# toonsegers/verifiable_mpc

Hardware: AMD Instinct MI355X
Metric: Ed25519 MSM scalar-mults/sec (higher is better)
Workload: dtype u32 (255-bit modular integers as 10 limbs of 25.5 bits, 32x32->64 multiply-adds)

## Files before the change

verifiable_mpc_amd/csrc/api.hip:

```cpp
#include <stdlib.h>

#include "common.h"


thread_local char vmpc_err_buf[512] = {0};

__attribute__((constructor)) static void vmpc_hw_queues_default() { setenv("GPU_MAX_HW_QUEUES", "16", 0); }

int vmpc_fr_check_dev(vmpc_ctx *ctx, const void *v, size_t n);

extern "C" const char *vmpc_last_error(void) { return vmpc_err_buf; }

const char *vmpc_getenv_experimental(const char *name) {
    const char *on = getenv("VMPC_EXPERIMENTAL");
    return (on && atoi(on) != 0) ? getenv(name) : nullptr;
}

extern "C" int vmpc_backend_info(char *buf, size_t buflen) {
    int n = 0;
    hipError_t e = hipGetDeviceCount(&n);
    if (e != hipSuccess || n <= 0) {
        if (buf && buflen) snprintf(buf, buflen, "no HIP device (%s)", hipGetErrorString(e));
        return VMPC_E_NODEV;
    }
// ... 16 lines not shown
        snprintf(vmpc_err_buf, sizeof vmpc_err_buf, "no HIP device visible");
        return VMPC_E_NODEV;
    }
    if (device < 0 || device >= n) return VMPC_E_INVAL;
    VMPC_HIP_CHECK(hipSetDevice(device));
    vmpc_ctx *c = new vmpc_ctx();
    c->device = device;
    hipDeviceProp_t p;
    if (hipGetDeviceProperties(&p, device) == hipSuccess) {
        c->cu_count = p.multiProcessorCount;
        c->lds_optin = p.sharedMemPerBlockOptin ? p.sharedMemPerBlockOptin : p.sharedMemPerBlock;
    }
    hipError_t e = hipStreamCreateWithFlags(&c->stream, hipStreamNonBlocking);
    if (e != hipSuccess) {
        delete c;
        snprintf(vmpc_err_buf, sizeof vmpc_err_buf, "hipStreamCreate: %s", hipGetErrorString(e));
        return VMPC_E_HIP;
    }
    c->own_stream = true;
    e = hipMalloc((void **)&c->d_status, (VMPC_ST_WORDS + 16) * sizeof(uint32_t));
    if (e == hipSuccess) e = hipMemset(c->d_status, 0, (VMPC_ST_WORDS + 16) * sizeof(uint32_t));
    if (e != hipSuccess) {
        VMPC_IGNORE(hipStreamDestroy(c->stream));
        delete c;
        snprintf(vmpc_err_buf, sizeof vmpc_err_buf, "hipMalloc(status): %s", hipGetErrorString(e));
        return VMPC_E_HIP;
    }
    const char *w = getenv("VMPC_MSM_WINDOW");
    if (w) c->window_override = atoi(w);
    const char *fj = getenv("VMPC_FOLD_JUMP_DIGITS");
    if (fj && atoi(fj) == 4) c->fold_jump_digit_bits = 4;
    const char *sp = getenv("VMPC_SHORT_PATH");
    if (sp) c->short_path = atoi(sp) != 0;
    const char *bb = vmpc_getenv_experimental("VMPC_BUCKET_BLOCK");
    if (bb && atoi(bb) == 1024) c->bucket_block = 1024;
    const char *bw = vmpc_getenv_experimental("VMPC_BUCKET_WGS_PER_CU");
    if (bw && atoi(bw) >= 0) c->bucket_wgs_per_cu = atoi(bw);
    const char *sf = vmpc_getenv_experimental("VMPC_SORT_FINE_BITS");
    if (sf && atoi(sf) >= 0) c->sort_fine_bits = atoi(sf);
    const char *rc = vmpc_getenv_experimental("VMPC_REDUCE_MAX_CHUNKS");
    if (rc && atoi(rc) >= 256 && atoi(rc) <= 32768) c->reduce_max_chunks = atoi(rc);
    const char *ro = vmpc_getenv_experimental("VMPC_REDUCE_CHUNKS");
    if (ro && atoi(ro) >= 64 && atoi(ro) <= 32768 && (atoi(ro) & (atoi(ro) - 1)) == 0) c->reduce_chunks_override = atoi(ro);
    const char *rt = vmpc_getenv_experimental("VMPC_REDUCE_TREE");
    if (rt) c->reduce_tree = atoi(rt) != 0;
    const char *ss = vmpc_getenv_experimental("VMPC_SEG_SHIFT_MIN");
    if (ss && atoi(ss) <= 0 && atoi(ss) >= -5) c->seg_shift_min = atoi(ss);
    *out = c;
    return VMPC_OK;
}

extern "C" int vmpc_ctx_destroy(vmpc_ctx *ctx) {
    if (!ctx) return VMPC_E_INVAL;
    if (ctx->p4_pool_busy) {
        snprintf(vmpc_err_buf, sizeof vmpc_err_buf, "vmpc_ctx_destroy: a vmpc_p4 of this context is still alive");
        return VMPC_E_INVAL;
    }
    VMPC_IGNORE(hipSetDevice(ctx->device));
    VMPC_IGNORE(hipStreamSynchronize(ctx->stream));
    for (auto &s : ctx->stages)
        for (auto &pr : s.pending) {
            VMPC_IGNORE(hipEventDestroy(pr.first));
            VMPC_IGNORE(hipEventDestroy(pr.second));
        }
    for (auto e : ctx->event_pool) VMPC_IGNORE(hipEventDestroy(e));
    if (ctx->xevent) VMPC_IGNORE(hipEventDestroy(ctx->xevent));
    if (ctx->ev_sorted) VMPC_IGNORE(hipEventDestroy(ctx->ev_sorted));
    if (ctx->ev_bucketed) VMPC_IGNORE(hipEventDestroy(ctx->ev_bucketed));
// ... 431 lines not shown
```

verifiable_mpc_amd/csrc/bn256_impl.h:

```cpp
#pragma once
#include "common.h"
#include "msm_sort.h"
#include "sw256.h"
#include "bn256_curve.h"

#define BN_B2A_CANON                                                                           \
    { 0xdb6c6949u, 0x7774124bu, 0x96e598bbu, 0x5a0cdfc5u, 0x111033b1u, 0x90e7f281u, 0x1aa5abfbu,  \
      0x64984e1fu }
#define BN_B2B_CANON                                                                           \
    { 0xd6340f0au, 0x35a2de0au, 0x83455ef6u, 0x316f8daeu, 0x7026e2d0u, 0x5dd7fe12u, 0xbaa9f3ffu,  \
      0x0e5ee696u }
static const msm_modulus BN_ORDER = {{0x57ac7261u, 0x1a2ef45bu, 0xf82b3924u, 0x2e8d8e12u, 0x6184dc21u,
                                      0xaa6fecb8u, 0x4aa387f9u, 0x8fb501e3u}};

template <class C, class F>
__global__ void __launch_bounds__(MSM_BLOCK)
gk_prep(const uint32_t *__restrict__ pts, size_t n_total, uint32_t *__restrict__ entries) {
    size_t i = (size_t)blockIdx.x * blockDim.x + threadIdx.x;
    if (i >= n_total) return;
    aff<F> a = aff_load<F>(pts + (size_t)C::AFF_WORDS * i);
    C::entry_st(entries + (size_t)C::ENTRY_WORDS * i, a);
}

template <class C>
__global__ void __launch_bounds__(MSM_BLOCK)
gk_bucket(const uint32_t *__restrict__ entries, const uint32_t *__restrict__ sorted,
          const uint32_t *__restrict__ starts, const uint32_t *__restrict__ counts,
          const uint32_t *__restrict__ nseg, const uint32_t *__restrict__ seg_starts,
          const uint2 *__restrict__ tasks, const uint32_t *__restrict__ n_tasks, int nb1, int seg, int balanced,
          uint32_t *__restrict__ buckets, uint32_t *__restrict__ partial) {
    uint32_t t = blockIdx.x * blockDim.x + threadIdx.x;
    if (t >= *n_tasks) return;
    uint2 tk = tasks[t];
    uint32_t ci = tk.x, sidx = tk.y;
    const uint32_t ns = nseg[ci];
    uint32_t lo, len;
    msm_seg_range(counts[ci], ns, sidx, (uint32_t)seg, balanced, lo, len);
    lo += starts[ci];
    typename C::acc_t acc = C::identity();
    for (uint32_t j = 0; j < len; j++) {
        uint32_t e = sorted[lo + j];
        typename C::entry_t q = C::entry_ld(entries + (size_t)C::ENTRY_WORDS * (e & 0x7fffffffu));
        acc = C::madd(acc, q, (e >> 31) != 0);
    }
    if (ns == 1)
        C::acc_st(buckets + (size_t)C::ACC_WORDS * msm_bucket_slot(ci, nb1), acc);
    else
        C::acc_st(partial + (size_t)C::ACC_WORDS * (seg_starts[ci] + sidx), acc);
}

template <class C, class F>
__global__ void __launch_bounds__(MSM_BLOCK)
gk_finish_light(const uint32_t *__restrict__ heavy_list, const uint32_t *__restrict__ ctrl,
                const uint32_t *__restrict__ nseg, const uint32_t *__restrict__ seg_starts,
                const uint32_t *__restrict__ partial, int nb1, uint32_t *__restrict__ buckets) {
    const uint32_t n_heavy = ctrl[0];
    for (uint32_t h = blockIdx.x * blockDim.x + threadIdx.x; h < n_heavy; h += gridDim.x * blockDim.x) {
        uint32_t ci = heavy_list[h];
        uint32_t ns = nseg[ci];
        if (ns > MSM_FINISH_SERIAL) continue;
        const uint32_t *src = partial + (size_t)C::ACC_WORDS * seg_starts[ci];
        typename C::acc_t acc = C::acc_ld(src);
        for (uint32_t j = 1; j < ns; j++) acc = jac_add<F>(acc, C::acc_ld(src + (size_t)C::ACC_WORDS * j));
        C::acc_st(buckets + (size_t)C::ACC_WORDS * msm_bucket_slot(ci, nb1), acc);
    }
}

template <class C, class F>
__global__ void __launch_bounds__(MSM_BLOCK)
gk_finish(const uint32_t *__restrict__ heavy_list, const uint32_t *__restrict__ ctrl,
          const uint32_t *__restrict__ nseg, const uint32_t *__restrict__ seg_starts,
          const uint32_t *__restrict__ partial, int nb1, uint32_t *__restrict__ buckets) {
    __shared__ uint32_t lds[MSM_BLOCK * C::ACC_WORDS];
    if (ctrl[4] == 0) return;
    const uint32_t n_heavy = ctrl[0];
    for (uint32_t h = blockIdx.x; h < n_heavy; h += gridDim.x) {
        uint32_t ci = heavy_list[h];
        uint32_t ns = nseg[ci];
        if (ns <= MSM_FINISH_SERIAL) continue;
        const uint32_t *src = partial + (size_t)C::ACC_WORDS * seg_starts[ci];
        typename C::acc_t acc = jac_identity<F>();
// ... 164 lines not shown
    aff_store<F>(out + (size_t)C::AFF_WORDS * i, jac_to_affine<F>(acc));
}


static inline bool bn_reduce_split(const msm_plan &p) {
    return (size_t)p.chunks * p.W <= 32768 && p.chunks >= 512 && (p.chunks & (p.chunks - 1)) == 0 &&
           p.chunks % (MSM_BLOCK / 2) == 0;
}

template <class C, class F>
struct bn_kernels {
    static int prep(vmpc_ctx *ctx, const void *points, size_t n, uint32_t *entries);
    static int bucket(vmpc_ctx *ctx, const msm_plan &p, msm_ws &w, const uint32_t *entries);
    static int reduce(vmpc_ctx *ctx, const msm_plan &p, msm_ws &w);
    static int final(vmpc_ctx *ctx, const msm_plan &p, msm_ws &w, void *out_affine, void *out_jac);
    static int final_multi(vmpc_ctx *ctx, const msm_plan &p, msm_ws &w, void *out_jac, int K);
    static int table_build(vmpc_ctx *ctx, const void *points, size_t n, size_t stride, void *table);
    static int validate(vmpc_ctx *ctx, const void *points, size_t n, unsigned long long *d_bad);
    static int fixed_base(vmpc_ctx *ctx, const void *base_affine, const void *scalars, size_t n, void *out_affine);
};

template <class C, class F>
int bn_kernels<C, F>::prep(vmpc_ctx *ctx, const void *points, size_t n, uint32_t *entries) {
    gk_prep<C, F><<<(unsigned)((n + MSM_BLOCK - 1) / MSM_BLOCK), MSM_BLOCK, 0, ctx->stream>>>((const uint32_t *)points, n,
                                                                                              entries);
    VMPC_KERNEL_CHECK();
    return VMPC_OK;
}

template <class C, class F>
int bn_kernels<C, F>::bucket(vmpc_ctx *ctx, const msm_plan &p, msm_ws &w, const uint32_t *entries) {
    hipStream_t st = ctx->stream;
    gk_bucket<C><<<(unsigned)((w.t_max + MSM_BLOCK - 1) / MSM_BLOCK), MSM_BLOCK, 0, st>>>(
        entries, w.sorted, w.starts, w.counts, w.nseg, w.seg_starts, w.tasks, w.ctrl + 1, p.nb1,
        (int)msm_seg_len(p), p.balanced, w.buckets, w.seg_partial);
    VMPC_KERNEL_CHECK();
    gk_finish_light<C, F><<<2 * ctx->cu_count, MSM_BLOCK, 0, st>>>(w.heavy_list, w.ctrl, w.nseg, w.seg_starts,
                                                                  w.seg_partial, p.nb1, w.buckets);
    VMPC_KERNEL_CHECK();
    gk_finish<C, F><<<2 * ctx->cu_count, MSM_BLOCK, 0, st>>>(w.heavy_list, w.ctrl, w.nseg, w.seg_starts,
                                                            w.seg_partial, p.nb1, w.buckets);
    VMPC_KERNEL_CHECK();
    return VMPC_OK;
}

template <class C, class F>
int bn_kernels<C, F>::reduce(vmpc_ctx *ctx, const msm_plan &p, msm_ws &w) {
    if (bn_reduce_split(p)) {
        const int bits = msm_ilog2(p.chunks), hb = (23 * bits + 19) / 39;
        gk_reduce<C, F, 2><<<dim3(2 * p.red_blocks, p.W), MSM_BLOCK, 0, ctx->stream>>>(
            w.buckets, w.counts, p.nb, p.chunks, p.chunk_len, msm_ilog2(p.chunk_len), 2 * p.red_blocks, hb, w.partials);
    } else {
        gk_reduce<C, F, 1><<<dim3(p.red_blocks, p.W), MSM_BLOCK, 0, ctx->stream>>>(
            w.buckets, w.counts, p.nb, p.chunks, p.chunk_len, msm_ilog2(p.chunk_len), p.red_blocks, 0, w.partials);
    }
    VMPC_KERNEL_CHECK();
    return VMPC_OK;
}

template <class C, class F>
int bn_kernels<C, F>::final(vmpc_ctx *ctx, const msm_plan &p, msm_ws &w, void *out_affine, void *out_jac) {
    gk_final<C, F><<<1, 64, 0, ctx->stream>>>(w.partials, p.W, bn_reduce_split(p) ? 2 * p.red_blocks : p.red_blocks, p.c,
                                              (uint32_t *)out_affine, (uint32_t *)out_jac);
    VMPC_KERNEL_CHECK();
    return VMPC_OK;
}

template <class C, class F>
// ... 47 lines not shown
```

verifiable_mpc_amd/csrc/common.h:

```cpp
#pragma once
#include <hip/hip_runtime.h>
#include <stdint.h>
#include <stdio.h>
#include <string.h>

#include <string>
#include <vector>

#include "../../include/vmpc.h"

extern thread_local char vmpc_err_buf[512];

#define VMPC_HIP_CHECK(expr)                                                                  \
    do {                                                                                      \
        hipError_t _e = (expr);                                                               \
        if (_e != hipSuccess) {                                                               \
            snprintf(vmpc_err_buf, sizeof vmpc_err_buf, "%s:%d: %s -> %s", __FILE__, __LINE__, \
                     #expr, hipGetErrorString(_e));                                           \
            return VMPC_E_HIP;                                                                \
        }                                                                                     \
    } while (0)

#define VMPC_CHECK(expr)              \
    do {                              \
        int _r = (expr);              \
        if (_r != VMPC_OK) return _r; \
    } while (0)

#define VMPC_ST_NONCANON 0
#define VMPC_ST_SHORT_OVERFLOW 1
#define VMPC_ST_WORDS 4

struct vmpc_stage {
    const char *name;
    double ms = 0;
    uint64_t launches = 0;
    std::vector<std::pair<hipEvent_t, hipEvent_t>> pending;
};

struct vmpc_ctx {
    int device = 0;
    hipStream_t stream = nullptr;
    bool own_stream = false;
    void *ws = nullptr;
    size_t ws_bytes = 0;
    size_t ws_used = 0;
    uint32_t *d_status = nullptr;
    int window_override = 0;
    int bucket_block = 256;
    int bucket_wgs_per_cu = 0;
    int reduce_max_chunks = 32768;
    int reduce_chunks_override = 0;
    int short_path = 1;
    int short_backoff = 0;
    size_t lds_optin = 0;
    int fold_jump_digit_bits = 8;
    bool sort_wide_ready = false;
    bool short_ready = false;
    uint32_t *short_cursors = nullptr;
    int reduce_tree = 1;
    bool reduce_tree_ready = false;
    int seg_shift_min = -3;
    int sort_fine_bits = -1;
    int plan_fill_shift = 0;
    int cu_count = 256;
    hipEvent_t xevent = nullptr;
    hipStream_t bucket_stream = nullptr;
    hipEvent_t ev_sorted = nullptr, ev_bucketed = nullptr;
    hipStream_t stage_stream = nullptr;
    void *pin = nullptr;
    size_t pin_bytes = 0;
    hipEvent_t pin_event = nullptr;
    bool stream_waits = false;
    uint32_t *done_flag_dev = nullptr;
    uint32_t done_seq = 0;
    uint32_t p4_seq = 0;
    void *pin_out = nullptr;
    void *pin_out_dev = nullptr;
    void *p4_pool = nullptr;
    size_t p4_pool_bytes = 0;
    bool p4_pool_busy = false;
    void *p4_kblock = nullptr;
// ... 43 lines not shown
```

verifiable_mpc_amd/csrc/msm.hip:

```cpp
#include <stdlib.h>

#include "common.h"
#include "fe25519.h"
#include "fr.h"
#include "ge25519.h"
#include "scan.h"
#include "quad.h"
#include "msm_sort.h"
#include "ptio.h"

#ifndef MSM_NIELS_STRIDE
#define MSM_NIELS_STRIDE 24
#endif
#ifndef MSM_REDUCE_WAVES
#define MSM_REDUCE_WAVES 2
#endif

__global__ void __launch_bounds__(MSM_BLOCK)
k_msm_prep(const uint32_t *__restrict__ aff, size_t n_main, const uint32_t *__restrict__ aff_extra,
           size_t n_total, uint32_t *__restrict__ niels) {
    size_t i = (size_t)blockIdx.x * blockDim.x + threadIdx.x;
    if (i >= n_total) return;
    const uint32_t *src = (i < n_main) ? aff + 16 * i : aff_extra + 16 * (i - n_main);
    ge_aff a;
    a.x = fe_ld8(src);
    a.y = fe_ld8(src + 8);
    ge_niels q = ge_niels_from_affine(a);
    niels_st_line(niels + NIELS_WORDS * i, q);
}

__device__ __forceinline__ ge_niels niels_ld(const uint32_t *niels, uint32_t e) {
    return niels_ld_line(niels + NIELS_WORDS * (size_t)(e & 0x7fffffffu));
}

#ifndef MSM_IDX_BATCH
#define MSM_IDX_BATCH 4
#endif
#ifndef MSM_BUCKET_WAVES
#define MSM_BUCKET_WAVES 4
#endif
template <int BLOCK>
__global__ void __launch_bounds__(BLOCK, BLOCK == MSM_BLOCK ? MSM_BUCKET_WAVES : 1)
k_msm_bucket(const uint32_t *__restrict__ niels, const uint32_t *__restrict__ sorted,
             const uint32_t *__restrict__ starts, const uint32_t *__restrict__ counts,
             const uint32_t *__restrict__ nseg, const uint32_t *__restrict__ seg_starts,
             const uint2 *__restrict__ tasks, const uint32_t *__restrict__ n_tasks, int nb1, int seg, int balanced,
             uint32_t *__restrict__ buckets, uint32_t *__restrict__ partial) {
    const uint32_t n_live = *n_tasks;
    for (uint32_t t = blockIdx.x * blockDim.x + threadIdx.x; t < n_live; t += gridDim.x * blockDim.x) {
    uint2 tk = tasks[t];
    uint32_t ci = tk.x, sidx = tk.y;
    const uint32_t ns = nseg[ci];
    uint32_t lo, len;
    msm_seg_range(counts[ci], ns, sidx, (uint32_t)seg, balanced, lo, len);
    lo += starts[ci];
    ge_ext acc = ge_ext_identity();
    uint32_t ev[MSM_IDX_BATCH];
#pragma unroll
    for (int k = 0; k < MSM_IDX_BATCH; k++) ev[k] = sorted[lo + ((uint32_t)k < len ? (uint32_t)k : len - 1)];
    uint32_t e = ev[0];
    ge_niels q = niels_ld(niels, e);
    for (uint32_t j0 = 0; j0 < len; j0 += MSM_IDX_BATCH) {
        uint32_t en_v[MSM_IDX_BATCH];
#pragma unroll
        for (int k = 0; k < MSM_IDX_BATCH; k++) {
            const uint32_t jj = j0 + MSM_IDX_BATCH + (uint32_t)k;
            en_v[k] = sorted[lo + (jj < len ? jj : len - 1)];
        }
#pragma unroll
        for (int k = 0; k < MSM_IDX_BATCH; k++) {
            if (j0 + (uint32_t)k < len) {
                const uint32_t en = k + 1 < MSM_IDX_BATCH ? ev[k + 1 < MSM_IDX_BATCH ? k + 1 : 0] : en_v[0];
                ge_niels qn = niels_ld(niels, en);
                acc = ge_madd(acc, ge_niels_select_neg(q, (e >> 31) != 0));
                e = en;
                q = qn;
            }
        }
#pragma unroll
        for (int k = 0; k < MSM_IDX_BATCH; k++) ev[k] = en_v[k];
    }
    if (ns == 1)
        ext_st(buckets + EXT_WORDS * msm_bucket_slot(ci, nb1), acc);
    else
        ext_st(partial + EXT_WORDS * (size_t)(seg_starts[ci] + sidx), acc);
    }
}


__global__ void __launch_bounds__(MSM_BLOCK)
k_msm_bucket_finish(const uint32_t *__restrict__ heavy_list, const uint32_t *__restrict__ ctrl,
                    const uint32_t *__restrict__ nseg, const uint32_t *__restrict__ seg_starts,
                    const uint32_t *__restrict__ partial, int nb1, uint32_t *__restrict__ buckets) {
    __shared__ uint32_t lds[MSM_BLOCK * EXT_WORDS];
    const uint32_t half = gridDim.x / 2;
    const uint32_t n_heavy = ctrl[0];
    if (blockIdx.x < half) {
    for (uint32_t h = blockIdx.x * blockDim.x + threadIdx.x; h < n_heavy; h += half * blockDim.x) {
        uint32_t ci = heavy_list[h];
        uint32_t ns = nseg[ci];
        if (ns > MSM_FINISH_SERIAL) continue;
        const uint32_t *src = partial + EXT_WORDS * (size_t)seg_starts[ci];
        ge_ext acc = ext_ld(src);
        for (uint32_t j = 1; j < ns; j++) acc = ge_add(acc, ext_ld(src + EXT_WORDS * (size_t)j));
        ext_st(buckets + EXT_WORDS * msm_bucket_slot(ci, nb1), acc);
    }
    return;
    }
    if (ctrl[4] == 0) return;
    for (uint32_t h = blockIdx.x - half; h < n_heavy; h += half) {
        uint32_t ci = heavy_list[h];
        uint32_t ns = nseg[ci];
        if (ns <= MSM_FINISH_SERIAL) continue;
        const uint32_t *src = partial + EXT_WORDS * (size_t)seg_starts[ci];
        ge_ext acc = ge_ext_identity();
        for (uint32_t j = threadIdx.x; j < ns; j += blockDim.x) acc = ge_add(acc, ext_ld(src + EXT_WORDS * (size_t)j));
        ext_st(lds + EXT_WORDS * threadIdx.x, acc);
        __syncthreads();
// ... 186 lines not shown
    return VMPC_OK;
}

__global__ void __launch_bounds__(MSM_BLOCK)
k_points_validate(const uint32_t *__restrict__ aff, size_t n, unsigned long long *__restrict__ bad) {
    size_t i = (size_t)blockIdx.x * blockDim.x + threadIdx.x;
    if (i >= n) return;
    uint32_t wx[8], wy[8];
    load_u32x8(wx, aff + 16 * i);
    load_u32x8(wy, aff + 16 * i + 8);
    ge_aff a;
    a.x = fe_unpack(wx);
    a.y = fe_unpack(wy);
    bool ok = fe8_is_canonical(wx) && fe8_is_canonical(wy) && ge_aff_on_curve(a);
    if (!ok) atomicAdd(bad, 1ull);
}


static int msm_accumulate(vmpc_ctx *ctx, const msm_plan &p, msm_ws &w, const uint32_t *entries, void *out_ext,
                          void *out_affine) {
    const int batch = p.W / p.period;
    hipStream_t st = ctx->stream;
    hipStream_t bst = ctx->bucket_stream ? ctx->bucket_stream : st;
    if (ctx->bucket_stream) {
        VMPC_HIP_CHECK(hipEventRecord(ctx->ev_sorted, st));
        VMPC_HIP_CHECK(hipStreamWaitEvent(bst, ctx->ev_sorted, 0));
    }
    {
        ctx->stage_stream = ctx->bucket_stream;
        vmpc_stage_scope s(ctx, "msm_bucket");
        unsigned grid = (unsigned)((w.t_max + MSM_BLOCK - 1) / MSM_BLOCK);
        if (ctx->bucket_wgs_per_cu > 0 && (unsigned)(ctx->bucket_wgs_per_cu * ctx->cu_count) < grid)
            grid = (unsigned)(ctx->bucket_wgs_per_cu * ctx->cu_count);
        if (ctx->bucket_block == 1024) {
            k_msm_bucket<1024><<<(grid + 3) / 4, 1024, 0, bst>>>(
                entries, w.sorted, w.starts, w.counts, w.nseg, w.seg_starts, w.tasks, w.ctrl + 1, p.nb1,
                (int)msm_seg_len(p), p.balanced, w.buckets, w.seg_partial);
        } else {
            k_msm_bucket<MSM_BLOCK><<<grid, MSM_BLOCK, 0, bst>>>(
                entries, w.sorted, w.starts, w.counts, w.nseg, w.seg_starts, w.tasks, w.ctrl + 1, p.nb1,
                (int)msm_seg_len(p), p.balanced, w.buckets, w.seg_partial);
        }
        const hipError_t e = hipGetLastError();
        if (e != hipSuccess) {
            ctx->stage_stream = nullptr;
            VMPC_HIP_CHECK(e);
        }
    }
    ctx->stage_stream = nullptr;
    if (ctx->bucket_stream) {
        VMPC_HIP_CHECK(hipEventRecord(ctx->ev_bucketed, bst));
        VMPC_HIP_CHECK(hipStreamWaitEvent(st, ctx->ev_bucketed, 0));
    }
    {
        vmpc_stage_scope s(ctx, "msm_bucket_finish");
        k_msm_bucket_finish<<<4 * ctx->cu_count, MSM_BLOCK, 0, st>>>(w.heavy_list, w.ctrl, w.nseg,
                                                                    w.seg_starts, w.seg_partial, p.nb1,
                                                                    w.buckets);
        VMPC_KERNEL_CHECK();
    }
    const bool tree = ctx->reduce_tree && msm_reduce_tree_fits(p);
    const int tree_parts = tree ? msm_reduce_tree_split(p) : 1;
    const bool tree_is_final = tree && p.period == 1 && out_ext && !out_affine && tree_parts == 1;
    {
        vmpc_stage_scope s(ctx, "msm_reduce");
        if (tree) {
            VMPC_CHECK(msm_reduce_tree(ctx, p, w, st, tree_is_final ? out_ext : nullptr));
        } else {
            k_msm_reduce<<<dim3(p.red_blocks, p.W), MSM_BLOCK, 0, st>>>(
                w.buckets, w.counts, p.nb, p.chunks, p.chunk_len, msm_ilog2(p.chunk_len), p.red_blocks, w.partials);
            VMPC_KERNEL_CHECK();
        }
    }
    if (!tree_is_final) {
        vmpc_stage_scope s(ctx, "msm_final");
// ... 367 lines not shown
```

verifiable_mpc_amd/csrc/msm_sort.h:

```cpp
#pragma once
#include "common.h"

#define MSM_MAX_C 16
#define MSM_WIDE_C 20
#define MSM_WIDE_ROWS 13
#define MSM_BLOCK 256
#define MSM_SORT_BLOCK 1024
#define MSM_SEG 64
#define MSM_SEG_LOG2 6
#define MSM_FINISH_SERIAL 32
#ifndef MSM_REDUCE_CHUNKS
#define MSM_REDUCE_CHUNKS 4096
#endif

struct msm_plan {
    size_t n_main, n_extra, n_total;
    int scalar_bits;
    int c, W, nb, nb1;
    int seg_shift;
    int balanced;
    int LB;
    int NC;
    int J;
    int idx_bits;
    int fine_in_entry;
    int period;
    int top_row;
    uint32_t top_max_b;
    int LB_top;
    size_t n_pad;
    int chunks;
    int chunk_len;
    int red_blocks;
    int wide = 0;
    int chunks_per_row = 0;
    int col_bits = 0;
    size_t row_stride = 0;
    int fine_cap = 12288;
};
inline size_t msm_seg_len(const msm_plan &p) { return (size_t)1 << (MSM_SEG_LOG2 + p.seg_shift); }


struct msm_ws {
    uint32_t *entries;
    uint32_t *hist1;
    size_t hist1_n;
    uint32_t *stage1;
    uint32_t *counts, *starts, *sorted;
    uint32_t *buckets;
    uint32_t *partials;
    uint32_t *nseg, *seg_starts, *block_hist, *block_base, *heavy_list, *ctrl;
    uint32_t *seg_partial;
    uint2 *tasks;
    int16_t *digits;
    void *scan_ws;
    size_t total;
    uint32_t plan_blocks;
    size_t t_max;
};

struct msm_modulus {
    uint32_t v[8];
};

void msm_make_plan(vmpc_ctx *ctx, size_t n_main, size_t n_extra, int scalar_bits, msm_plan &p,
                   const msm_modulus *modulus = nullptr);
void msm_plan_geometry(vmpc_ctx *ctx, msm_plan &p);
void msm_layout(const msm_plan &p, msm_ws &w, char *base, size_t entry_bytes, size_t acc_bytes);
bool msm_reduce_tree_fits(const msm_plan &p);
int msm_reduce_tree_split(const msm_plan &p);
int msm_reduce_tree(vmpc_ctx *ctx, const msm_plan &p, msm_ws &w, hipStream_t st, void *out_packed);
int msm_sort_stage(vmpc_ctx *ctx, const msm_plan &p, msm_ws &w, const void *scalars, size_t n,
                   const void *extra_scalars, const msm_modulus &modulus);
int msm_sort_digits(vmpc_ctx *ctx, const msm_plan &p, msm_ws &w);
int msm_recode_wide_batch(vmpc_ctx *ctx, const void *const *scalars, size_t n_main, const void *const *extra_scalars,
                          int K, size_t extra_pos, size_t n_extra, size_t row_stride, int32_t *digits32,
                          size_t digits_per_commitment, const msm_modulus &modulus);
int msm_recode_rows(vmpc_ctx *ctx, const void *scalars, size_t n_main, const void *extra_scalars,
                    size_t extra_pos, size_t n_extra, size_t n_pad, int16_t *digits, int c, int W, int rows,
                    const msm_modulus &modulus);
int msm_recode_rows_batch(vmpc_ctx *ctx, const void *const *scalars, size_t n_main, const void *const *extra_scalars,
                          int K, size_t extra_pos, size_t n_extra, size_t n_pad, int16_t *digits,
                          size_t digits_per_commitment, int c, int W, int rows, const msm_modulus &modulus);

static inline int msm_ilog2(int v) {
    int r = 0;
    while ((1 << r) < v) r++;
    return r;
}

__host__ __device__ __forceinline__ uint32_t msm_seg_count(uint32_t cnt, uint32_t seg_log) {
    return (cnt + (1u << seg_log) - 1u) >> seg_log;
}
__device__ __forceinline__ void msm_seg_range(uint32_t cnt, uint32_t ns, uint32_t sidx, uint32_t seg, int balanced,
                                              uint32_t &off, uint32_t &len) {
    if (ns <= 1) {
        off = 0;
        len = cnt;
        return;
    }
    if (!balanced) {
        off = sidx * seg;
        len = cnt - off < seg ? cnt - off : seg;
        return;
    }
    const uint32_t q = cnt / ns, r = cnt - q * ns;
    off = sidx * q + (sidx < r ? sidx : r);
    len = q + (sidx < r ? 1u : 0u);
}

__device__ __forceinline__ size_t msm_bucket_slot(uint32_t ci, int nb1) {
    uint32_t w = ci / (uint32_t)nb1;
    return (size_t)ci - w - 1;
}
```

verifiable_mpc_amd/csrc/msm_sort.hip:

```cpp
#include "common.h"
#include "msm_sort.h"
#include "scan.h"

#define SORT_T 8192
#define SORT_BLOCK 1024
#define SORT_WAVES (SORT_BLOCK / 64)
#define SORT_FINE_CAP 12288

__device__ __forceinline__ uint32_t msm_seg_class(uint32_t rem, int seg_shift) {
    return seg_shift > 0 ? (rem + (1u << seg_shift) - 1u) >> seg_shift : rem;
}

__device__ __forceinline__ void load_u32x8(uint32_t dst[8], const uint32_t *src) {
    const uint4 *p = reinterpret_cast<const uint4 *>(src);
    uint4 a = p[0], b = p[1];
    dst[0] = a.x; dst[1] = a.y; dst[2] = a.z; dst[3] = a.w;
    dst[4] = b.x; dst[5] = b.y; dst[6] = b.z; dst[7] = b.w;
}

struct msm_recode_batch {
    const uint32_t *sc[16];
    const uint32_t *sc_extra[16];
};

// ... 522 lines not shown
__device__ __forceinline__ void msm_classes_body(uint32_t *__restrict__ ctrl, int W, uint32_t *__restrict__ class_base,
                                                 uint32_t *scratch) {
    const int ncell = MSM_SEG * W;
    uint32_t running = 0;
    for (int k0 = 0; k0 < ncell; k0 += 1024) {
        const int k = k0 + (int)threadIdx.x;
        uint32_t v = k < ncell ? ctrl[16 + k] : 0u, tot;
        uint32_t ex = vmpc_block_excl_scan<uint32_t>(v, &tot, scratch);
        if (k < ncell) class_base[k] = running + ex;
        running += tot;
    }
    if (threadIdx.x == 0) ctrl[1] = running;
}

__global__ void __launch_bounds__(1024)
k_msm_classes(uint32_t *__restrict__ ctrl, int W, uint32_t *__restrict__ class_base) {
    __shared__ uint32_t scratch[16];
    msm_classes_body(ctrl, W, class_base, scratch);
}

__global__ void __launch_bounds__(1024)
k_msm_ranks_classes(uint32_t *__restrict__ block_hist, int NC, int W, uint32_t *__restrict__ ctrl,
                    uint32_t *__restrict__ class_base) {
    __shared__ uint32_t part[16][MSM_SEG];
    __shared__ uint32_t scratch[16];
    for (int w = 0; w < W; w++) {
        msm_ranks_window(block_hist, NC, W, w, ctrl, part);
        __syncthreads();
    }
    msm_classes_body(ctrl, W, class_base, scratch);
}

__global__ void __launch_bounds__(512)
k_msm_plan2(const uint32_t *__restrict__ counts, int NC, int W, int NF, int top_row, int period, int NF_top, int nb1,
            int seg_shift, int balanced,
            const uint32_t *__restrict__ class_base, const uint32_t *__restrict__ block_rank,
            uint2 *__restrict__ tasks) {
    const uint32_t seg_log = (uint32_t)(MSM_SEG_LOG2 + seg_shift);
    __shared__ uint32_t cur[MSM_SEG + 1], first[MSM_SEG + 1];
    const uint32_t block = blockIdx.x;
    const int w = block / NC, cb = block % NC;
    if (threadIdx.x >= 1 && threadIdx.x <= MSM_SEG) {
        cur[threadIdx.x] = 0;
        first[threadIdx.x] = class_base[(MSM_SEG - threadIdx.x) * W + w] +
                             block_rank[(size_t)block * MSM_SEG + (threadIdx.x - 1)];
    }
    __syncthreads();
    if (w % period == top_row) NF = NF_top;
    if (threadIdx.x >= (unsigned)NF) return;
    const size_t ci = (size_t)w * nb1 + 1 + (size_t)cb * NF + threadIdx.x;
    const uint32_t cnt = counts[ci];
    const uint32_t ns = msm_seg_count(cnt, seg_log);
    if (balanced) {
        if (ns) {
            const uint32_t bin = msm_seg_class((cnt + ns - 1u) / ns, seg_shift);
            const uint32_t base = first[bin] + atomicAdd(&cur[bin], ns);
            for (uint32_t sidx = 0; sidx < ns; sidx++) tasks[base + sidx] = make_uint2((uint32_t)ci, sidx);
        }
        return;
    }
    const uint32_t full = cnt >> seg_log, rem = cnt & ((1u << seg_log) - 1u);
    if (rem) {
        const uint32_t bin = msm_seg_class(rem, seg_shift);
        tasks[first[bin] + atomicAdd(&cur[bin], 1u)] = make_uint2((uint32_t)ci, full);
    }
    if (full) {
        const uint32_t base = first[MSM_SEG] + atomicAdd(&cur[MSM_SEG], full);
        for (uint32_t sidx = 0; sidx < full; sidx++) tasks[base + sidx] = make_uint2((uint32_t)ci, sidx);
    }
}

static int msm_pick_window(size_t n, int scalar_bits) {
    if (scalar_bits == 253) return n > (1u << 13) ? 16 : 11;
    double best = 1e300;
    int best_c = 4;
    for (int c = 4; c <= MSM_MAX_C; c++) {
        int W = (scalar_bits + 2 + c - 1) / c;
        double cost = (double)W * ((double)n + 2.5 * (double)(1u << (c - 1)));
        if (cost < best) {
            best = cost;
            best_c = c;
        }
    }
    return best_c;
}

static uint32_t msm_top_max_bucket(const msm_modulus &mod, int c, int W) {
    uint32_t m1[8];
    uint64_t borrow = 1;
    for (int i = 0; i < 8; i++) {
        uint64_t v = (uint64_t)mod.v[i] - borrow;
        m1[i] = (uint32_t)v;
        borrow = (v >> 63) & 1;
    }
    const int shift = c * (W - 1);
    if (shift >= 256) return 0;
    uint64_t top = 0;
    for (int bit = 0; bit < 32 && shift + bit < 256; bit++)
        top |= (uint64_t)((m1[(shift + bit) >> 5] >> ((shift + bit) & 31)) & 1u) << bit;
    for (int bit = shift + 32; bit < 256; bit++)
        if ((m1[bit >> 5] >> (bit & 31)) & 1u) return 0xffffffffu;
// ... 72 lines not shown
    p.chunk_len = p.nb / chunks;
    p.red_blocks = (chunks + MSM_BLOCK - 1) / MSM_BLOCK;
}

void msm_layout(const msm_plan &p, msm_ws &w, char *base, size_t entry_bytes, size_t acc_bytes) {
    size_t off = 0;
    auto take = [&](size_t bytes) {
        size_t o = off;
        off += vmpc_align(bytes);
        return base ? (void *)(base + o) : (void *)nullptr;
    };
    size_t nbk = (size_t)p.W * p.nb1;
    w.entries = (uint32_t *)take(p.n_total * entry_bytes);
    w.digits = (int16_t *)take((size_t)p.W * p.n_pad * (p.wide ? 4 : 2));
    w.hist1_n = (size_t)p.W * p.NC * p.J;
    w.hist1 = (uint32_t *)take((w.hist1_n + 1) * 4);
    w.counts = (uint32_t *)take(nbk * 4);
    w.starts = (uint32_t *)take(nbk * 4);
    w.stage1 = (uint32_t *)take((size_t)p.W * p.n_total * 4);
    w.sorted = (uint32_t *)take((size_t)p.W * p.n_total * 4);
    w.buckets = (uint32_t *)take((size_t)p.W * p.nb * acc_bytes);
    w.partials = (uint32_t *)take((size_t)p.W * (3 * p.red_blocks + 4) * acc_bytes);
    size_t m_max = (size_t)p.W * p.n_total;
    size_t nonempty_max = m_max < (size_t)p.W * p.nb ? m_max : (size_t)p.W * p.nb;
    w.t_max = m_max / msm_seg_len(p) + nonempty_max;
    w.plan_blocks = (uint32_t)(p.W * p.NC);
    size_t hist_n = (size_t)MSM_SEG * w.plan_blocks;
    w.block_hist = (uint32_t *)take(hist_n * 4);
    w.block_base = (uint32_t *)take((size_t)MSM_SEG * p.W * 4);
    w.nseg = (uint32_t *)take(nbk * 4);
    w.seg_starts = (uint32_t *)take(nbk * 4);
    w.heavy_list = (uint32_t *)take(nbk * 4);
    w.ctrl = (uint32_t *)take((16 + (size_t)MSM_SEG * p.W) * 4);
    w.tasks = (uint2 *)take(w.t_max * 8);
    w.seg_partial = (uint32_t *)take(w.t_max * acc_bytes);
    size_t scan_n = hist_n;
    if (w.hist1_n > scan_n) scan_n = w.hist1_n;
    w.scan_ws = take(vmpc_scan_ws_bytes(scan_n, 4));
    w.total = off;
}

int msm_sort_stage(vmpc_ctx *ctx, const msm_plan &p, msm_ws &w, const void *scalars, size_t n,
                   const void *extra_scalars, const msm_modulus &modulus) {
    hipStream_t st = ctx->stream;
    const size_t n_total = p.n_total;
    const unsigned gb = (unsigned)((p.n_pad + MSM_BLOCK - 1) / MSM_BLOCK);
    {
        vmpc_stage_scope s(ctx, "msm_recode");
        k_msm_recode<<<gb, MSM_BLOCK, 0, st>>>((const uint32_t *)scalars, n,
                                              (const uint32_t *)extra_scalars, n, n_total - n, p.n_pad, w.digits, p.c,
                                              p.W, p.W, p.n_pad, modulus, ctx->d_status);
        VMPC_KERNEL_CHECK();
    }
    return msm_sort_digits(ctx, p, w);
}

int msm_recode_rows(vmpc_ctx *ctx, const void *scalars, size_t n_main, const void *extra_scalars,
                    size_t extra_pos, size_t n_extra, size_t n_pad, int16_t *digits, int c, int W, int rows,
                    const msm_modulus &modulus) {
    vmpc_stage_scope s(ctx, "msm_recode");
    const int wpr = W / rows;
    k_msm_recode<<<(unsigned)((n_pad + MSM_BLOCK - 1) / MSM_BLOCK), MSM_BLOCK, 0, ctx->stream>>>(
        (const uint32_t *)scalars, n_main, (const uint32_t *)extra_scalars, extra_pos, n_extra, n_pad, digits, c,
        W, wpr, (size_t)rows * n_pad, modulus, ctx->d_status);
    VMPC_KERNEL_CHECK();
    return VMPC_OK;
}
// ... 81 lines not shown
            if (lds_bytes > 48 * 1024)
                VMPC_HIP_CHECK(hipFuncSetAttribute((const void *)k_sort_part1<true>,
                                                   hipFuncAttributeMaxDynamicSharedMemorySize, (int)lds_bytes));
            k_sort_part1<true><<<chunk_grid, SORT_BLOCK, lds_bytes, st>>>(
                w.digits, p.n_pad, p.NC, p.LB, p.top_row, p.period, p.LB_top, p.J, p.idx_bits, p.chunks_per_row, xcd,
                w.hist1, w.stage1);
        } else {
            if (lds_bytes > 48 * 1024)
                VMPC_HIP_CHECK(hipFuncSetAttribute((const void *)k_sort_part1<false>,
                                                   hipFuncAttributeMaxDynamicSharedMemorySize, (int)lds_bytes));
            k_sort_part1<false><<<chunk_grid, SORT_BLOCK, lds_bytes, st>>>(
                w.digits, p.n_pad, p.NC, p.LB, p.top_row, p.period, p.LB_top, p.J, p.fine_in_entry ? p.idx_bits : 31, 0, 0,
                w.hist1, w.stage1);
        }
        VMPC_KERNEL_CHECK();
    }
    {
        vmpc_stage_scope s(ctx, "msm_sort");
        if (p.wide) VMPC_CHECK((msm_launch_fine<true, 16384>(ctx, p, w)));
        else if (p.fine_in_entry) VMPC_CHECK((msm_launch_fine<true, SORT_FINE_CAP>(ctx, p, w)));
        else VMPC_CHECK((msm_launch_fine<false, SORT_FINE_CAP>(ctx, p, w)));
    }
    {
        vmpc_stage_scope s(ctx, "msm_plan");
        if (p.W <= 8 && (size_t)p.W * p.NC <= 1024) {
            k_msm_ranks_classes<<<1, 1024, 0, st>>>(w.block_hist, p.NC, p.W, w.ctrl, w.block_base);
            VMPC_KERNEL_CHECK();
        } else {
            k_msm_ranks<<<p.W, 1024, 0, st>>>(w.block_hist, p.NC, p.W, w.ctrl);
            VMPC_KERNEL_CHECK();
            k_msm_classes<<<1, 1024, 0, st>>>(w.ctrl, p.W, w.block_base);
            VMPC_KERNEL_CHECK();
        }
        k_msm_plan2<<<w.plan_blocks, 512, 0, st>>>(w.counts, p.NC, p.W, 1 << p.LB, p.top_row, p.period, 1 << p.LB_top,
                                                  p.nb1, p.seg_shift, p.balanced, w.block_base, w.block_hist, w.tasks);
        VMPC_KERNEL_CHECK();
    }
    return VMPC_OK;
}
```

Before: 1.378 billion.

## Precompute bucket task ranges in planner and stage sorted indices in LDS

The planner kernel now writes fully resolved tasks (start offset, length, destination slot, split flag) as uint4. The bucket kernels no longer do the dependent lookups of counts, starts, nseg and seg_starts or compute segment ranges. The Ed25519 bucket kernel also copies each task's run of sorted indices into a per-thread column in shared memory, 32 at a time, instead of prefetching them from global memory in small register batches. The 1024-thread bucket block option is removed. The costs are doubled task storage, 32 KB of LDS per block that may limit occupancy, and extra fill loops for long runs.

```diff
diff --git a/verifiable_mpc_amd/csrc/api.hip b/verifiable_mpc_amd/csrc/api.hip
--- a/verifiable_mpc_amd/csrc/api.hip
+++ b/verifiable_mpc_amd/csrc/api.hip
@@ -72,8 +72,6 @@
     if (fj && atoi(fj) == 4) c->fold_jump_digit_bits = 4;
     const char *sp = getenv("VMPC_SHORT_PATH");
     if (sp) c->short_path = atoi(sp) != 0;
-    const char *bb = vmpc_getenv_experimental("VMPC_BUCKET_BLOCK");
-    if (bb && atoi(bb) == 1024) c->bucket_block = 1024;
     const char *bw = vmpc_getenv_experimental("VMPC_BUCKET_WGS_PER_CU");
     if (bw && atoi(bw) >= 0) c->bucket_wgs_per_cu = atoi(bw);
     const char *sf = vmpc_getenv_experimental("VMPC_SORT_FINE_BITS");
diff --git a/verifiable_mpc_amd/csrc/bn256_impl.h b/verifiable_mpc_amd/csrc/bn256_impl.h
--- a/verifiable_mpc_amd/csrc/bn256_impl.h
+++ b/verifiable_mpc_amd/csrc/bn256_impl.h
@@ -25,28 +25,19 @@
 template <class C>
 __global__ void __launch_bounds__(MSM_BLOCK)
 gk_bucket(const uint32_t *__restrict__ entries, const uint32_t *__restrict__ sorted,
-          const uint32_t *__restrict__ starts, const uint32_t *__restrict__ counts,
-          const uint32_t *__restrict__ nseg, const uint32_t *__restrict__ seg_starts,
-          const uint2 *__restrict__ tasks, const uint32_t *__restrict__ n_tasks, int nb1, int seg, int balanced,
+          const msm_task *__restrict__ tasks, const uint32_t *__restrict__ n_tasks,
           uint32_t *__restrict__ buckets, uint32_t *__restrict__ partial) {
     uint32_t t = blockIdx.x * blockDim.x + threadIdx.x;
     if (t >= *n_tasks) return;
-    uint2 tk = tasks[t];
-    uint32_t ci = tk.x, sidx = tk.y;
-    const uint32_t ns = nseg[ci];
-    uint32_t lo, len;
-    msm_seg_range(counts[ci], ns, sidx, (uint32_t)seg, balanced, lo, len);
-    lo += starts[ci];
+    const msm_task tk = tasks[t];
+    const uint32_t lo = tk.x, len = tk.y;
     typename C::acc_t acc = C::identity();
     for (uint32_t j = 0; j < len; j++) {
         uint32_t e = sorted[lo + j];
         typename C::entry_t q = C::entry_ld(entries + (size_t)C::ENTRY_WORDS * (e & 0x7fffffffu));
         acc = C::madd(acc, q, (e >> 31) != 0);
     }
-    if (ns == 1)
-        C::acc_st(buckets + (size_t)C::ACC_WORDS * msm_bucket_slot(ci, nb1), acc);
-    else
-        C::acc_st(partial + (size_t)C::ACC_WORDS * (seg_starts[ci] + sidx), acc);
+    C::acc_st(((tk.w & MSM_TASK_SPLIT) ? partial : buckets) + (size_t)C::ACC_WORDS * tk.z, acc);
 }
 
 template <class C, class F>
@@ -277,8 +268,7 @@
 int bn_kernels<C, F>::bucket(vmpc_ctx *ctx, const msm_plan &p, msm_ws &w, const uint32_t *entries) {
     hipStream_t st = ctx->stream;
     gk_bucket<C><<<(unsigned)((w.t_max + MSM_BLOCK - 1) / MSM_BLOCK), MSM_BLOCK, 0, st>>>(
-        entries, w.sorted, w.starts, w.counts, w.nseg, w.seg_starts, w.tasks, w.ctrl + 1, p.nb1,
-        (int)msm_seg_len(p), p.balanced, w.buckets, w.seg_partial);
+        entries, w.sorted, w.tasks, w.ctrl + 1, w.buckets, w.seg_partial);
     VMPC_KERNEL_CHECK();
     gk_finish_light<C, F><<<2 * ctx->cu_count, MSM_BLOCK, 0, st>>>(w.heavy_list, w.ctrl, w.nseg, w.seg_starts,
                                                                   w.seg_partial, p.nb1, w.buckets);
diff --git a/verifiable_mpc_amd/csrc/common.h b/verifiable_mpc_amd/csrc/common.h
--- a/verifiable_mpc_amd/csrc/common.h
+++ b/verifiable_mpc_amd/csrc/common.h
@@ -47,7 +47,6 @@
     size_t ws_used = 0;
     uint32_t *d_status = nullptr;
     int window_override = 0;
-    int bucket_block = 256;
     int bucket_wgs_per_cu = 0;
     int reduce_max_chunks = 32768;
     int reduce_chunks_override = 0;
diff --git a/verifiable_mpc_amd/csrc/msm.hip b/verifiable_mpc_amd/csrc/msm.hip
--- a/verifiable_mpc_amd/csrc/msm.hip
+++ b/verifiable_mpc_amd/csrc/msm.hip
@@ -33,57 +33,51 @@
     return niels_ld_line(niels + NIELS_WORDS * (size_t)(e & 0x7fffffffu));
 }
 
-#ifndef MSM_IDX_BATCH
-#define MSM_IDX_BATCH 4
-#endif
 #ifndef MSM_BUCKET_WAVES
 #define MSM_BUCKET_WAVES 4
 #endif
-template <int BLOCK>
-__global__ void __launch_bounds__(BLOCK, BLOCK == MSM_BLOCK ? MSM_BUCKET_WAVES : 1)
+#define MSM_IDX_WIN 32
+template <int N>
+__device__ __forceinline__ void msm_idx_fill(uint32_t *__restrict__ col, const uint32_t *__restrict__ src, uint32_t n) {
+    uint32_t v[N];
+#pragma unroll
+    for (int k = 0; k < N; k++) v[k] = (uint32_t)k < n ? src[k] : 0u;
+#pragma unroll
+    for (int k = 0; k < N; k++) col[k * MSM_BLOCK] = v[k];
+}
+
+__global__ void __launch_bounds__(MSM_BLOCK, MSM_BUCKET_WAVES)
 k_msm_bucket(const uint32_t *__restrict__ niels, const uint32_t *__restrict__ sorted,
-             const uint32_t *__restrict__ starts, const uint32_t *__restrict__ counts,
-             const uint32_t *__restrict__ nseg, const uint32_t *__restrict__ seg_starts,
-             const uint2 *__restrict__ tasks, const uint32_t *__restrict__ n_tasks, int nb1, int seg, int balanced,
+             const msm_task *__restrict__ tasks, const uint32_t *__restrict__ n_tasks,
              uint32_t *__restrict__ buckets, uint32_t *__restrict__ partial) {
+    __shared__ uint32_t idx_stage[MSM_IDX_WIN * MSM_BLOCK];
+    uint32_t *const col = idx_stage + threadIdx.x;
     const uint32_t n_live = *n_tasks;
     for (uint32_t t = blockIdx.x * blockDim.x + threadIdx.x; t < n_live; t += gridDim.x * blockDim.x) {
-    uint2 tk = tasks[t];
-    uint32_t ci = tk.x, sidx = tk.y;
-    const uint32_t ns = nseg[ci];
-    uint32_t lo, len;
-    msm_seg_range(counts[ci], ns, sidx, (uint32_t)seg, balanced, lo, len);
-    lo += starts[ci];
+    const msm_task tk = tasks[t];
+    const uint32_t *run = sorted + tk.x;
+    const uint32_t len = tk.y;
+    if (len <= 8) msm_idx_fill<8>(col, run, len);
+    else msm_idx_fill<MSM_IDX_WIN>(col, run, len);
     ge_ext acc = ge_ext_identity();
-    uint32_t ev[MSM_IDX_BATCH];
-#pragma unroll
-    for (int k = 0; k < MSM_IDX_BATCH; k++) ev[k] = sorted[lo + ((uint32_t)k < len ? (uint32_t)k : len - 1)];
-    uint32_t e = ev[0];
-    ge_niels q = niels_ld(niels, e);
-    for (uint32_t j0 = 0; j0 < len; j0 += MSM_IDX_BATCH) {
-        uint32_t en_v[MSM_IDX_BATCH];
-#pragma unroll
-        for (int k = 0; k < MSM_IDX_BATCH; k++) {
-            const uint32_t jj = j0 + MSM_IDX_BATCH + (uint32_t)k;
-            en_v[k] = sorted[lo + (jj < len ? jj : len - 1)];
-        }
-#pragma unroll
-        for (int k = 0; k < MSM_IDX_BATCH; k++) {
-            if (j0 + (uint32_t)k < len) {
-                const uint32_t en = k + 1 < MSM_IDX_BATCH ? ev[k + 1 < MSM_IDX_BATCH ? k + 1 : 0] : en_v[0];
-                ge_niels qn = niels_ld(niels, en);
-                acc = ge_madd(acc, ge_niels_select_neg(q, (e >> 31) != 0));
-                e = en;
-                q = qn;
-            }
-        }
-#pragma unroll
-        for (int k = 0; k < MSM_IDX_BATCH; k++) ev[k] = en_v[k];
-    }
-    if (ns == 1)
-        ext_st(buckets + EXT_WORDS * msm_bucket_slot(ci, nb1), acc);
-    else
-        ext_st(partial + EXT_WORDS * (size_t)(seg_starts[ci] + sidx), acc);
+    for (uint32_t left = len;;) {
+        const uint32_t n = left < MSM_IDX_WIN ? left : MSM_IDX_WIN;
+        uint32_t e = col[0];
+        ge_niels q = niels_ld(niels, e);
+        for (uint32_t k = 0; k < n; k++) {
+            const uint32_t en = col[(k + 1 < n ? k + 1 : k) * MSM_BLOCK];
+            ge_niels qn = niels_ld(niels, en);
+            acc = ge_madd(acc, ge_niels_select_neg(q, (e >> 31) != 0));
+            e = en;
+            q = qn;
+        }
+        if (left <= MSM_IDX_WIN) break;
+        left -= MSM_IDX_WIN;
+        run += MSM_IDX_WIN;
+        for (uint32_t k0 = 0; k0 < MSM_IDX_WIN && k0 < left; k0 += 8)
+            msm_idx_fill<8>(col + k0 * MSM_BLOCK, run + k0, left - k0);
+    }
+    ext_st(((tk.w & MSM_TASK_SPLIT) ? partial : buckets) + EXT_WORDS * (size_t)tk.z, acc);
     }
 }
 
@@ -336,15 +330,7 @@
         unsigned grid = (unsigned)((w.t_max + MSM_BLOCK - 1) / MSM_BLOCK);
         if (ctx->bucket_wgs_per_cu > 0 && (unsigned)(ctx->bucket_wgs_per_cu * ctx->cu_count) < grid)
             grid = (unsigned)(ctx->bucket_wgs_per_cu * ctx->cu_count);
-        if (ctx->bucket_block == 1024) {
-            k_msm_bucket<1024><<<(grid + 3) / 4, 1024, 0, bst>>>(
-                entries, w.sorted, w.starts, w.counts, w.nseg, w.seg_starts, w.tasks, w.ctrl + 1, p.nb1,
-                (int)msm_seg_len(p), p.balanced, w.buckets, w.seg_partial);
-        } else {
-            k_msm_bucket<MSM_BLOCK><<<grid, MSM_BLOCK, 0, bst>>>(
-                entries, w.sorted, w.starts, w.counts, w.nseg, w.seg_starts, w.tasks, w.ctrl + 1, p.nb1,
-                (int)msm_seg_len(p), p.balanced, w.buckets, w.seg_partial);
-        }
+        k_msm_bucket<<<grid, MSM_BLOCK, 0, bst>>>(entries, w.sorted, w.tasks, w.ctrl + 1, w.buckets, w.seg_partial);
         const hipError_t e = hipGetLastError();
         if (e != hipSuccess) {
             ctx->stage_stream = nullptr;
diff --git a/verifiable_mpc_amd/csrc/msm_sort.h b/verifiable_mpc_amd/csrc/msm_sort.h
--- a/verifiable_mpc_amd/csrc/msm_sort.h
+++ b/verifiable_mpc_amd/csrc/msm_sort.h
@@ -41,6 +41,9 @@
 inline size_t msm_seg_len(const msm_plan &p) { return (size_t)1 << (MSM_SEG_LOG2 + p.seg_shift); }
 
 
+typedef uint4 msm_task;
+#define MSM_TASK_SPLIT 1u
+
 struct msm_ws {
     uint32_t *entries;
     uint32_t *hist1;
@@ -51,7 +54,7 @@
     uint32_t *partials;
     uint32_t *nseg, *seg_starts, *block_hist, *block_base, *heavy_list, *ctrl;
     uint32_t *seg_partial;
-    uint2 *tasks;
+    msm_task *tasks;
     int16_t *digits;
     void *scan_ws;
     size_t total;
@@ -113,3 +116,11 @@
     uint32_t w = ci / (uint32_t)nb1;
     return (size_t)ci - w - 1;
 }
+
+__device__ __forceinline__ msm_task msm_make_task(uint32_t ci, uint32_t start, uint32_t cnt, uint32_t ns, uint32_t sidx,
+                                                  uint32_t seg, int balanced, uint32_t seg_start, int nb1) {
+    uint32_t off, len;
+    msm_seg_range(cnt, ns, sidx, seg, balanced, off, len);
+    if (ns <= 1) return make_uint4(start + off, len, (uint32_t)msm_bucket_slot(ci, nb1), 0u);
+    return make_uint4(start + off, len, seg_start + sidx, MSM_TASK_SPLIT);
+}
diff --git a/verifiable_mpc_amd/csrc/msm_sort.hip b/verifiable_mpc_amd/csrc/msm_sort.hip
--- a/verifiable_mpc_amd/csrc/msm_sort.hip
+++ b/verifiable_mpc_amd/csrc/msm_sort.hip
@@ -578,10 +578,11 @@
 }
 
 __global__ void __launch_bounds__(512)
-k_msm_plan2(const uint32_t *__restrict__ counts, int NC, int W, int NF, int top_row, int period, int NF_top, int nb1,
+k_msm_plan2(const uint32_t *__restrict__ counts, const uint32_t *__restrict__ starts,
+            const uint32_t *__restrict__ seg_starts, int NC, int W, int NF, int top_row, int period, int NF_top, int nb1,
             int seg_shift, int balanced,
             const uint32_t *__restrict__ class_base, const uint32_t *__restrict__ block_rank,
-            uint2 *__restrict__ tasks) {
+            msm_task *__restrict__ tasks) {
     const uint32_t seg_log = (uint32_t)(MSM_SEG_LOG2 + seg_shift);
     __shared__ uint32_t cur[MSM_SEG + 1], first[MSM_SEG + 1];
     const uint32_t block = blockIdx.x;
@@ -597,22 +598,26 @@
     const size_t ci = (size_t)w * nb1 + 1 + (size_t)cb * NF + threadIdx.x;
     const uint32_t cnt = counts[ci];
     const uint32_t ns = msm_seg_count(cnt, seg_log);
+    if (ns == 0) return;
+    const uint32_t start = starts[ci], seg = 1u << seg_log;
+    const uint32_t seg_start = ns > 1 ? seg_starts[ci] : 0u;
     if (balanced) {
-        if (ns) {
-            const uint32_t bin = msm_seg_class((cnt + ns - 1u) / ns, seg_shift);
-            const uint32_t base = first[bin] + atomicAdd(&cur[bin], ns);
-            for (uint32_t sidx = 0; sidx < ns; sidx++) tasks[base + sidx] = make_uint2((uint32_t)ci, sidx);
-        }
+        const uint32_t bin = msm_seg_class((cnt + ns - 1u) / ns, seg_shift);
+        const uint32_t base = first[bin] + atomicAdd(&cur[bin], ns);
+        for (uint32_t sidx = 0; sidx < ns; sidx++)
+            tasks[base + sidx] = msm_make_task((uint32_t)ci, start, cnt, ns, sidx, seg, 1, seg_start, nb1);
         return;
     }
-    const uint32_t full = cnt >> seg_log, rem = cnt & ((1u << seg_log) - 1u);
+    const uint32_t full = cnt >> seg_log, rem = cnt & (seg - 1u);
     if (rem) {
         const uint32_t bin = msm_seg_class(rem, seg_shift);
-        tasks[first[bin] + atomicAdd(&cur[bin], 1u)] = make_uint2((uint32_t)ci, full);
+        tasks[first[bin] + atomicAdd(&cur[bin], 1u)] =
+            msm_make_task((uint32_t)ci, start, cnt, ns, full, seg, 0, seg_start, nb1);
     }
     if (full) {
         const uint32_t base = first[MSM_SEG] + atomicAdd(&cur[MSM_SEG], full);
-        for (uint32_t sidx = 0; sidx < full; sidx++) tasks[base + sidx] = make_uint2((uint32_t)ci, sidx);
+        for (uint32_t sidx = 0; sidx < full; sidx++)
+            tasks[base + sidx] = msm_make_task((uint32_t)ci, start, cnt, ns, sidx, seg, 0, seg_start, nb1);
     }
 }
 
@@ -751,7 +756,7 @@
     w.seg_starts = (uint32_t *)take(nbk * 4);
     w.heavy_list = (uint32_t *)take(nbk * 4);
     w.ctrl = (uint32_t *)take((16 + (size_t)MSM_SEG * p.W) * 4);
-    w.tasks = (uint2 *)take(w.t_max * 8);
+    w.tasks = (msm_task *)take(w.t_max * sizeof(msm_task));
     w.seg_partial = (uint32_t *)take(w.t_max * acc_bytes);
     size_t scan_n = hist_n;
     if (w.hist1_n > scan_n) scan_n = w.hist1_n;
@@ -899,8 +904,9 @@
             k_msm_classes<<<1, 1024, 0, st>>>(w.ctrl, p.W, w.block_base);
             VMPC_KERNEL_CHECK();
         }
-        k_msm_plan2<<<w.plan_blocks, 512, 0, st>>>(w.counts, p.NC, p.W, 1 << p.LB, p.top_row, p.period, 1 << p.LB_top,
-                                                  p.nb1, p.seg_shift, p.balanced, w.block_base, w.block_hist, w.tasks);
+        k_msm_plan2<<<w.plan_blocks, 512, 0, st>>>(w.counts, w.starts, w.seg_starts, p.NC, p.W, 1 << p.LB, p.top_row,
+                                                  p.period, 1 << p.LB_top, p.nb1, p.seg_shift, p.balanced, w.block_base,
+                                                  w.block_hist, w.tasks);
         VMPC_KERNEL_CHECK();
     }
     return VMPC_OK;
```

New measurement: 1.414 billion (median of 6 runs). 2.6% higher.
